# j-wilson/GPflowPILCO

Measured on AMD Instinct MI355X. Metric: moment_matched_rollout_step_elements_per_sec, higher is better.
Workload: dtype f32; 1 GPU; C3 (BASELINE configs[2]): N=2000 d=8 D=8 H=40 fp32 drift moment-match step / closed rollout; recipe=baseline: BASELINE.md recipe: lengthscales log-U[0.3,3], GP-prior targets, fresh mu~U[0,1]^d / Sigm~; N=2000, d=8, D=8, H=40, B_per_gpu=256, B_total=256, B_this_rank=256, parallelism=dp1 over B (weak), recipe=baseline, steps_requested=418, diag_pairs=f64, offdiag_pairs=f32

## Files before the change

gpflowpilco_amd/_lib.py:

```python
from __future__ import annotations

import ctypes as C
import os

_HERE = os.path.dirname(os.path.abspath(__file__))
LIB_PATH = os.environ.get("GPFLOWPILCO_MM_LIB") or os.path.join(_HERE, "libgpflowpilco_mm.so")

MM_F32, MM_F64 = 0, 1
MM_DMAX = 32
MM_M_ALIGN = 128
MM_FULL_OUTPUT_COV = 1
MM_MODEL_UNCERTAINTY = 2
MM_FORCE_GENERIC = 4
MM_STAGE_DIAG = 8
MM_STAGE_OFFDIAG = 16
MM_STAGE_FINALIZE = 32
MM_FORCE_WORST_TIER = 64
MM_WORKSPACE_CURRENT = 128
MM_FORCE_ROUTE = 256
MM_NO_ROUTE = 512
MM_SUMS_CURRENT = 1024
MM_ISTAGE_OLD_SKIP_BOUND = 1 << 26
MM_ISTAGE_NO_BOUND_SKIP = 1 << 27

ERRORS = {
    -1: "MM_E_ARG: NULL pointer or non-positive size",
    -2: "MM_E_DIM: input dimension d exceeds MM_DMAX=32 or unsupported shape",
    -3: "MM_E_DTYPE: dtype must be MM_F32 or MM_F64",
    -4: "MM_E_WORKSPACE: workspace/packed buffer too small",
    -5: "MM_E_NO_C: model_uncertainty requested but the model was packed without C",
    -6: "MM_E_STATE: Euler update / closed rollout needs d == L and a full output covariance",
}

SIGNATURES = {
    "mm_abi_version": (C.c_int, []),
    "mm_packed_model_bytes": (C.c_size_t, [C.c_int] * 5),
    "mm_pack_model": (C.c_int, [C.c_void_p, C.c_size_t, C.c_int, C.c_int, C.c_int, C.c_int]
                      + [C.c_void_p] * 6 + [C.c_void_p]),
    "mm_pack_perm": (C.c_int, [C.c_void_p, C.c_size_t, C.c_int, C.c_int, C.c_int, C.c_int, C.c_void_p, C.c_void_p]),
    "mm_workspace_bytes": (C.c_size_t, [C.c_int] * 6),
    "mm_moment_match": (C.c_int, [C.c_void_p, C.c_size_t, C.c_int, C.c_int, C.c_int, C.c_int, C.c_int,
                                  C.c_void_p, C.c_void_p, C.c_int, C.c_double,
                                  C.c_void_p, C.c_void_p, C.c_void_p,
                                  C.c_void_p, C.c_size_t, C.c_void_p, C.c_void_p]),
    "mm_q_forward": (C.c_int, [C.c_void_p, C.c_size_t, C.c_int, C.c_int, C.c_int, C.c_int, C.c_int,
                               C.c_void_p, C.c_void_p, C.c_int,
                               C.c_void_p, C.c_void_p, C.c_void_p,
                               C.c_void_p, C.c_size_t, C.c_void_p, C.c_void_p]),
    "mm_Q_reduce_forward": (C.c_int, [C.c_void_p, C.c_size_t, C.c_int, C.c_int, C.c_int, C.c_int, C.c_int,
                                      C.c_int, C.c_double, C.c_void_p,
                                      C.c_void_p, C.c_size_t, C.c_void_p]),
    "mm_euler_update": (C.c_int, [C.c_int, C.c_int, C.c_int, C.c_double] + [C.c_void_p] * 8),
    "mm_expected_cost": (C.c_int, [C.c_int, C.c_int, C.c_int] + [C.c_void_p] * 6),
    "mm_offdiag_stats": (C.c_int, [C.c_void_p, C.c_size_t, C.c_int, C.c_int, C.c_int, C.c_int, C.c_int, C.c_int,
                                   C.c_void_p, C.c_size_t, C.c_void_p, C.c_void_p]),
    "mm_offdiag_worklist_len": (C.c_int, [C.c_int] * 6 + [C.c_void_p, C.c_size_t, C.c_void_p, C.c_void_p]),
    "mm_offdiag_skip_bounds": (C.c_int, [C.c_void_p, C.c_size_t, C.c_int, C.c_int, C.c_int, C.c_int, C.c_int, C.c_int,
                                         C.c_void_p, C.c_size_t, C.c_void_p, C.c_void_p, C.c_void_p]),
    "mm_route_estimates": (C.c_int, [C.c_void_p, C.c_size_t, C.c_int, C.c_int, C.c_int, C.c_int, C.c_int, C.c_int,
                                     C.c_void_p, C.c_size_t, C.c_void_p, C.c_void_p]),
    "mm_compose_workspace_bytes": (C.c_size_t, [C.c_int] * 4),
    "mm_compose_nd_workspace_bytes": (C.c_size_t, [C.c_int] * 5),
    "mm_compose_tape_bytes": (C.c_size_t, [C.c_int] * 6),
    "mm_compose_backward_workspace_bytes": (C.c_size_t, [C.c_int] * 4),
    "mm_policy_grad_bytes": (C.c_size_t, [C.c_int] * 3),
    "mm_compose_tape_bytes_nd": (C.c_size_t, [C.c_int] * 7),
    "mm_compose_backward_workspace_bytes_nd": (C.c_size_t, [C.c_int] * 6),
    "mm_policy_grad_bytes_nd": (C.c_size_t, [C.c_int] * 4),
    "mm_compose_nd_mixed_workspace_bytes": (C.c_size_t, [C.c_int] * 6),
    "mm_compose_tape_bytes_nd_mixed": (C.c_size_t, [C.c_int] * 8),
    "mm_compose_backward_workspace_bytes_nd_mixed": (C.c_size_t, [C.c_int] * 7),
    "mm_bwd_f32_supported": (C.c_int, [C.c_int]),
    "mm_backward_pair_aggregates_bytes": (C.c_size_t, [C.c_int] * 5),
    "mm_backward_pair_aggregates": (C.c_int, [C.c_void_p, C.c_size_t, C.c_int, C.c_int, C.c_int, C.c_int, C.c_int,
                                              C.c_void_p, C.c_void_p, C.c_int, C.c_void_p, C.c_size_t, C.c_void_p, C.c_size_t,
                                              C.c_void_p, C.c_size_t, C.c_void_p, C.c_void_p]),
    "mm_moment_match_backward_bytes": (C.c_size_t, [C.c_int] * 5),
    "mm_moment_match_backward_bytes_dtype": (C.c_size_t, [C.c_int] * 6),
    "mm_moment_match_backward": (C.c_int, [C.c_void_p, C.c_size_t, C.c_int, C.c_int, C.c_int, C.c_int, C.c_int,
                                           C.c_void_p, C.c_void_p, C.c_int,
                                           C.c_void_p, C.c_void_p, C.c_void_p,
                                           C.c_void_p, C.c_void_p, C.c_int,
                                           C.c_void_p, C.c_size_t, C.c_void_p, C.c_size_t,
                                           C.c_void_p, C.c_void_p]),
    "mm_moment_match_with_sums": (C.c_int, [C.c_void_p, C.c_size_t, C.c_int, C.c_int, C.c_int, C.c_int, C.c_int,
                                            C.c_void_p, C.c_void_p, C.c_int, C.c_double,
                                            C.c_void_p, C.c_void_p, C.c_void_p,
                                            C.c_void_p, C.c_size_t, C.c_void_p, C.c_size_t,
                                            C.c_void_p, C.c_void_p]),
    "mm_backward_bytes": (C.c_size_t, [C.c_int] * 5),
    "mm_backward_sums": (C.c_int, [C.c_void_p, C.c_size_t, C.c_int, C.c_int, C.c_int, C.c_int, C.c_int,
                                   C.c_void_p, C.c_int, C.c_void_p, C.c_size_t, C.c_void_p, C.c_size_t, C.c_void_p]),
    "mm_pathwise_eval": (C.c_int, [C.c_int] * 6 + [C.c_void_p] * 12),
    "mm_pathwise_rollout": (C.c_int, [C.c_int] * 7 + [C.c_double] + [C.c_void_p] * 13),
    "mm_pathwise_eval_jac": (C.c_int, [C.c_int] * 6 + [C.c_void_p] * 13),
    "mm_pathwise_eval_bound": (C.c_int, [C.c_int] * 6 + [C.c_void_p] * 13),
    "mm_pathwise_tape_bytes": (C.c_size_t, [C.c_int] * 6),
    "mm_pathwise_policy_rollout": (C.c_int, [C.c_int] * 5 + [C.c_double, C.c_int, C.c_int] + [C.c_void_p] * 10
                                   + [C.c_void_p, C.c_size_t, C.c_int, C.c_double, C.c_double]
                                   + [C.c_void_p] * 4 + [C.c_void_p, C.c_size_t, C.c_int, C.c_void_p]),
    "mm_pathwise_backward_scratch_bytes": (C.c_size_t, [C.c_int] * 3),
    "mm_pathwise_policy_rollout_backward": (C.c_int, [C.c_int] * 3 + [C.c_double, C.c_int, C.c_int, C.c_void_p]
                                            + [C.c_void_p, C.c_size_t, C.c_int, C.c_double, C.c_double]
                                            + [C.c_void_p] * 2 + [C.c_void_p, C.c_size_t] + [C.c_void_p] * 3
                                            + [C.c_void_p, C.c_size_t, C.c_void_p]),
    "mm_pathwise_policy_rollout_backward_seeded": (C.c_int, [C.c_int] * 3 + [C.c_double, C.c_int, C.c_int, C.c_void_p]
                                                   + [C.c_void_p, C.c_size_t, C.c_int, C.c_double, C.c_double]
                                                   + [C.c_void_p] * 2 + [C.c_void_p, C.c_size_t] + [C.c_void_p] * 4
                                                   + [C.c_void_p, C.c_size_t, C.c_void_p]),
    "mm_pathwise_tape_bytes_nd": (C.c_size_t, [C.c_int] * 7),
    "mm_pathwise_policy_rollout_nd": (C.c_int, [C.c_int] * 5 + [C.c_double, C.c_int, C.c_int, C.c_void_p, C.c_int]
                                      + [C.c_void_p] * 9
                                      + [C.c_void_p, C.c_size_t, C.c_int, C.c_void_p, C.c_void_p]
                                      + [C.c_void_p] * 4 + [C.c_void_p, C.c_size_t, C.c_int, C.c_void_p]),
    "mm_pathwise_backward_scratch_bytes_nd": (C.c_size_t, [C.c_int] * 4),
    "mm_pathwise_policy_rollout_backward_nd": (C.c_int, [C.c_int] * 3 + [C.c_double, C.c_int, C.c_int, C.c_void_p, C.c_int]
                                               + [C.c_void_p, C.c_size_t, C.c_int, C.c_void_p, C.c_void_p]
                                               + [C.c_void_p] * 2 + [C.c_void_p, C.c_size_t] + [C.c_void_p] * 3
                                               + [C.c_void_p, C.c_size_t, C.c_void_p]),
    "mm_pathwise_policy_rollout_backward_nd_seeded": (C.c_int, [C.c_int] * 3 + [C.c_double, C.c_int, C.c_int, C.c_void_p, C.c_int]
                                                      + [C.c_void_p, C.c_size_t, C.c_int, C.c_void_p, C.c_void_p]
                                                      + [C.c_void_p] * 2 + [C.c_void_p, C.c_size_t] + [C.c_void_p] * 4
                                                      + [C.c_void_p, C.c_size_t, C.c_void_p]),
    "mm_pathwise_policy_rollout_wide": (C.c_int, [C.c_int] * 5 + [C.c_double, C.c_int, C.c_int, C.c_void_p, C.c_int]
                                        + [C.c_void_p] * 9
                                        + [C.c_void_p, C.c_size_t, C.c_int, C.c_void_p, C.c_void_p]
                                        + [C.c_void_p] * 4 + [C.c_void_p, C.c_size_t, C.c_int, C.c_void_p]),
    "mm_pathwise_backward_scratch_bytes_wide": (C.c_size_t, [C.c_int] * 4),
    "mm_pathwise_policy_rollout_backward_wide": (C.c_int, [C.c_int] * 3 + [C.c_double, C.c_int, C.c_int, C.c_void_p, C.c_int]
                                                 + [C.c_void_p, C.c_size_t, C.c_int, C.c_void_p, C.c_void_p]
                                                 + [C.c_void_p] * 2 + [C.c_void_p, C.c_size_t] + [C.c_void_p] * 3
                                                 + [C.c_void_p, C.c_size_t, C.c_void_p]),
    "mm_pathwise_policy_rollout_backward_wide_seeded": (C.c_int, [C.c_int] * 3 + [C.c_double, C.c_int, C.c_int, C.c_void_p, C.c_int]
                                                        + [C.c_void_p, C.c_size_t, C.c_int, C.c_void_p, C.c_void_p]
                                                        + [C.c_void_p] * 2 + [C.c_void_p, C.c_size_t] + [C.c_void_p] * 4
                                                        + [C.c_void_p, C.c_size_t, C.c_void_p]),
    "mm_pathwise_tape_bytes_mixed": (C.c_size_t, [C.c_int] * 8),
    "mm_pathwise_policy_rollout_mixed": (C.c_int, [C.c_int] * 5 + [C.c_double, C.c_int, C.c_int, C.c_void_p, C.c_int]
                                         + [C.c_void_p] * 9
                                         + [C.c_void_p, C.c_size_t, C.c_int, C.c_void_p, C.c_void_p]
                                         + [C.c_void_p] * 4 + [C.c_void_p, C.c_size_t, C.c_int, C.c_void_p]
                                         + [C.c_int, C.c_void_p, C.c_void_p]),
    "mm_pathwise_policy_rollout_backward_mixed": (C.c_int, [C.c_int] * 3 + [C.c_double, C.c_int, C.c_int, C.c_void_p, C.c_int]
                                                  + [C.c_void_p, C.c_size_t, C.c_int, C.c_void_p, C.c_void_p]
                                                  + [C.c_void_p] * 2 + [C.c_void_p, C.c_size_t] + [C.c_void_p] * 4
                                                  + [C.c_void_p, C.c_size_t, C.c_void_p] + [C.c_int, C.c_void_p]),
    "mm_pathwise_eval_kern": (C.c_int, [C.c_int] * 6 + [C.c_void_p] * 12 + [C.c_int]),
    "mm_pathwise_rollout_kern": (C.c_int, [C.c_int] * 7 + [C.c_double] + [C.c_void_p] * 13 + [C.c_int]),
    "mm_pathwise_eval_jac_kern": (C.c_int, [C.c_int] * 6 + [C.c_void_p] * 13 + [C.c_int]),
    "mm_pathwise_eval_bound_kern": (C.c_int, [C.c_int] * 6 + [C.c_void_p] * 13 + [C.c_int]),
    "mm_pathwise_policy_rollout_kern": (C.c_int, [C.c_int] * 5 + [C.c_double, C.c_int, C.c_int, C.c_void_p, C.c_int]
                                        + [C.c_void_p] * 9
                                        + [C.c_void_p, C.c_size_t, C.c_int, C.c_void_p, C.c_void_p]
                                        + [C.c_void_p] * 4 + [C.c_void_p, C.c_size_t, C.c_int, C.c_void_p]
                                        + [C.c_int, C.c_void_p, C.c_void_p, C.c_int]),
    "mm_pathwise_mean_eval": (C.c_int, [C.c_int] * 5 + [C.c_void_p] * 10 + [C.c_int]),
    "mm_pathwise_policy_rollout_mean": (C.c_int, [C.c_int] * 4 + [C.c_double, C.c_int, C.c_int, C.c_void_p, C.c_int]
                                        + [C.c_void_p] * 6
                                        + [C.c_void_p, C.c_size_t, C.c_int, C.c_void_p, C.c_void_p]
                                        + [C.c_void_p] * 4 + [C.c_void_p, C.c_size_t, C.c_int, C.c_void_p]
                                        + [C.c_int, C.c_void_p, C.c_void_p, C.c_int]),
    "mm_pathwise_basis": (C.c_int, [C.c_int] * 5 + [C.c_void_p] * 9),
    "mm_pathwise_pack_stream": (C.c_int, [C.c_int] * 5 + [C.c_void_p] * 4),
    "mm_gram_workspace_bytes": (C.c_size_t, [C.c_int] * 4),
    "mm_gram_se": (C.c_int, [C.c_int] * 4 + [C.c_void_p] * 6),
    "mm_gram_se_backward": (C.c_int, [C.c_int] * 4 + [C.c_void_p] * 9 + [C.c_size_t, C.c_void_p]),
    "mm_predict_workspace_bytes": (C.c_size_t, [C.c_int] * 4),
    "mm_predict_se": (C.c_int, [C.c_int] * 4 + [C.c_void_p] * 10 + [C.c_size_t, C.c_void_p]),
    "mm_rollout_closed": (C.c_int, [C.c_void_p, C.c_size_t, C.c_int, C.c_int, C.c_int, C.c_int, C.c_int, C.c_int,
                                    C.c_double, C.c_int, C.c_double,
                                    C.c_void_p, C.c_void_p, C.c_void_p, C.c_void_p,
                                    C.c_void_p, C.c_size_t, C.c_void_p, C.c_void_p]),
}


def _composed_rollout_signatures():
# ... 65 lines not shown
```

gpflowpilco_amd/csrc/mm_common.h:

```cpp
#pragma once
#include <stddef.h>
#include <stdint.h>
#include "../../include/gpflowpilco_mm.h"

static inline size_t mm_align_up(size_t x, size_t a) { return (x + a - 1) / a * a; }
static inline int mm_round_up_int(int x, int a) { return (x + a - 1) / a * a; }
static inline size_t mm_elem_size(int dtype) { return dtype == MM_F64 ? 8 : 4; }

#define MM_ISTAGE_NO_ROUTE (1 << 20)
#define MM_ISTAGE_ROUTE (1 << 21)
#define MM_ISTAGE_NO_M56 (1 << 22)
#define MM_ISTAGE_OLD_OFFDIAG (1 << 23)
#define MM_ISTAGE_OLD_SPOLY56 (1 << 24)
#define MM_ISTAGE_OLD_DIAG_MAP (1 << 25)
#define MM_ISTAGE_OLD_SKIP_BOUND (1 << 26)
#define MM_ISTAGE_NO_BOUND_SKIP (1 << 27)

#define MM_PW_KERNELS 3

static inline int mm_num_pairs(int L, int flags) {
  return (flags & MM_FULL_OUTPUT_COV) ? L * (L + 1) / 2 : L;
}

static inline int mm_moment_deg(int d) { return d <= 8 ? 4 : 2; }
static inline long long mm_binom(int n, int k) {
  if (k < 0 || k > n) return 0;
  long long r = 1;
  for (int i = 1; i <= k; ++i) r = r * (n - k + i) / i;
  return r;
}
static inline int mm_mono_count(int n, int d) { return (int)mm_binom(d + n - 1, n); }
static inline int mm_mono_offset(int n, int d) { int o = 0; for (int m = 0; m < n; ++m) o += mm_mono_count(m, d); return o; }
static inline size_t mm_rank_table_entries(int d) {
  const int dk = d <= 8 ? 8 : 32, deg = mm_moment_deg(d);
  size_t n = 0, p = 1;
  for (int k = 1; k <= deg; ++k) { p *= dk; n += p; }
  return n;
}
static inline int mm_moment_cols(int d) { return mm_round_up_int(mm_mono_offset(mm_moment_deg(d) + 1, d), 16); }
static inline int mm_moment56_off5(int d) { return d <= 8 ? mm_round_up_int(mm_mono_count(4, d), 128) : 0; }
static inline int mm_moment56_off6(int d) { return d <= 8 ? mm_moment56_off5(d) + mm_round_up_int(mm_mono_count(5, d), 128) : 0; }
static inline int mm_moment56_cols(int d) { return d <= 8 ? mm_moment56_off6(d) + mm_round_up_int(mm_mono_count(6, d), 128) : 0; }
struct MMTab56 { int ins[6], last[6], n_i16, mult2, mult3, n_f32; size_t bytes; };
static inline MMTab56 mm_tab56(int d) {
  MMTab56 t;
  int o = 0;
  for (int m = 0; m < 6; ++m) { t.ins[m] = o; o += mm_mono_count(m, d) * 8; }
  for (int k = 0; k < 6; ++k) { t.last[k] = o; o += mm_mono_count(k, d); }
  t.n_i16 = mm_round_up_int(o, 8);
  t.mult2 = 0; t.mult3 = mm_mono_count(2, d); t.n_f32 = mm_mono_count(2, d) + mm_mono_count(3, d);
  t.bytes = (size_t)t.n_i16 * 2 + (size_t)t.n_f32 * 4;
  return t;
}

struct MMModelLayout {
  int Mp, Kz, nd8, KMp;
  size_t Z64;
  size_t Zt64;
  size_t zbar;
  size_t ls2;
  size_t var;
  size_t meanc;
  size_t beta64;
  size_t Zc64;
  size_t Zc;
  size_t Zs3;
  size_t Zm;
  size_t zmax2;
  size_t rtab;
  size_t Zq2;
  size_t Zm56;
  size_t tab56;
  size_t perm;
  size_t skey;
  size_t zt2;
  size_t zt2s;
  size_t Cm;
  size_t total;
};
#define MM_SORT_MIN_M 256

static inline MMModelLayout mm_model_layout(int L, int M, int d, int dtype, int with_C) {
  MMModelLayout o;
  const size_t es = mm_elem_size(dtype), A = 256;
  o.Mp = mm_round_up_int(M, MM_M_ALIGN);
  o.Kz = mm_round_up_int(d, 2);
  o.nd8 = (d + 7) / 8;
  o.KMp = mm_moment_cols(d);
  size_t off = 0;
  o.Z64 = off;    off = mm_align_up(off + (size_t)L * M * d * 8, A);
  o.Zt64 = off;   off = mm_align_up(off + (size_t)L * d * o.Mp * 8, A);
  o.zbar = off;   off = mm_align_up(off + (size_t)L * d * 8, A);
  o.ls2 = off;    off = mm_align_up(off + (size_t)L * d * 8, A);
  o.var = off;    off = mm_align_up(off + (size_t)L * 8, A);
  o.meanc = off;  off = mm_align_up(off + (size_t)L * 8, A);
  o.beta64 = off; off = mm_align_up(off + (size_t)L * M * 8, A);
  o.Zc64 = off;   off = mm_align_up(off + (size_t)L * o.Mp * o.Kz * 8, A);
  o.Zc = o.Zc64;
  if (dtype != MM_F64) { o.Zc = off; off = mm_align_up(off + (size_t)L * o.Mp * o.Kz * es, A); }
  o.Zs3 = off;
  if (dtype != MM_F64) off = mm_align_up(off + (size_t)L * o.Mp * 24 * o.nd8 * 2, A);
  o.Zm = off;
  if (dtype != MM_F64) off = mm_align_up(off + (size_t)L * o.Mp * o.KMp * 8, A);
  o.zmax2 = off;  off = mm_align_up(off + (size_t)L * 8, A);
  o.rtab = off;   off = mm_align_up(off + mm_rank_table_entries(d) * 2, A);
  o.Zq2 = off;
  if (dtype != MM_F64 && d <= 8) off = mm_align_up(off + (size_t)L * (o.Mp / 32) * 8192, A);
  o.Zm56 = off;
  if (dtype != MM_F64 && d <= 8) off = mm_align_up(off + (size_t)L * 2 * mm_moment56_cols(d) * o.Mp * 2, A);
  o.tab56 = off;
  if (dtype != MM_F64 && d <= 8) off = mm_align_up(off + mm_tab56(d).bytes, A);
  o.perm = off;   off = mm_align_up(off + (size_t)L * o.Mp * 4, A);
  o.skey = off;   off = mm_align_up(off + (size_t)L * o.Mp * 8, A);
  o.zt2 = off;    off = mm_align_up(off + (size_t)L * (o.Mp / 32) * 4, A);
  o.zt2s = off;   off = mm_align_up(off + (size_t)L * (o.Mp / 32) * 4, A);
  o.Cm = off;
  if (with_C) off = mm_align_up(off + (size_t)L * o.Mp * o.Mp * 8, A);
  o.total = off;
  return o;
}

#define MM_MOM_SPLIT 2
#ifndef MM_COLLAPSE_BOUND2
#define MM_COLLAPSE_BOUND2 0.25f
#endif
#define MM_C6_X5_2 (1.0f / 256.0f)
#define MM_C6_X4_2 (1.0f / 1600.0f)
#define MM_C6_MAX 0.25f
#define MM_C6_C0 1.666663289e-01f
#define MM_C6_C1 4.166659713e-02f
#define MM_C6_C2 8.350561373e-03f
#define MM_C6_C3 1.391559141e-03f
#define MM_C6_SYS2 6.33e-6f
#define MM_C6_POLY_F64(x_) (((x_) * (x_)) * (x_) * fma(fma(fma((double)MM_C6_C3, (x_), (double)MM_C6_C2), (x_), (double)MM_C6_C1), (x_), (double)MM_C6_C0))
#ifndef MM_TIER1_DIV
#define MM_TIER1_DIV 20
#endif
#if MM_TIER1_DIV == 16
#define MM_TIER1_MAX 0.0625f
#define MM_REM1_C0 1.666936278e-01f
#define MM_REM1_C1 4.167173430e-02f
#elif MM_TIER1_DIV == 20
#define MM_TIER1_MAX 0.05f
#define MM_REM1_C0 1.666839272e-01f
#define MM_REM1_C1 4.166988656e-02f
#elif MM_TIER1_DIV == 24
#define MM_TIER1_MAX 0.041666668f
#define MM_REM1_C0 1.666786522e-01f
#define MM_REM1_C1 4.166889191e-02f
#elif MM_TIER1_DIV == 32
#define MM_TIER1_MAX 0.03125f
#define MM_REM1_C0 1.666734070e-01f
#define MM_REM1_C1 4.166791216e-02f
#else
#error "MM_TIER1_DIV must be 16, 20, 24 or 32"
#endif
#define MM_INSIDE_BOUND2 (0.998f * MM_C6_MAX * MM_C6_MAX)
#ifndef MM_ROUTE_TOL
#define MM_ROUTE_TOL 3.0e-4
#endif
#define MM_ROUTE_CSPLIT 8
static inline int mm_route_ncc(int NS, int npanel) { int n = NS / npanel; return n < 1 ? 1 : (n > MM_ROUTE_CSPLIT ? MM_ROUTE_CSPLIT : n); }
#define MM_EXP_CAP_F64 700.0
#define MM_EXP_CAP_F32 80.0f
#define MM_GEN_ROWS 64
#define MM_GEN_COLS 256
#define MM_PANEL_ROWS 256
__host__ __device__ inline int mm_mfma_groups(int Mp) { return (Mp + MM_PANEL_ROWS - 1) / MM_PANEL_ROWS * (MM_PANEL_ROWS / 64); }
__host__ __device__ inline int mm_f32p_list_off(int L) { return 4 + 2 * L; }
// ... 109 lines not shown
```

gpflowpilco_amd/csrc/mm_moments.hip:

```cpp
#include <hip/hip_runtime.h>
#include <math.h>
#include "mm_common.h"
#include "mm_mono.h"

typedef double f64x4m __attribute__((ext_vector_type(4)));

#define MM_GEMM_RB 64
#define MM_GEMM_NB 128
#define MM_GEMM_KB 32
#define MM_GEMM_AS 34
#define MM_GEMM_BS 144

__device__ __forceinline__ void mm_decode_pair_m(int p, int L, int& a, int& a2) {
  int r = p - L, i = 0;
  while (r >= L - 1 - i) { r -= L - 1 - i; ++i; }
  a = i; a2 = i + 1 + r;
}

__global__ __launch_bounds__(256) __attribute__((amdgpu_waves_per_eu(2, 2))) void k_wmom_gemm(const double* __restrict__ whR, const double* __restrict__ whC,
                                                      const double* __restrict__ Zm, int KMp, int L, int Mp, int B, int Po,
                                                      int nrb, int ncb, int nwork, int col_deg3,
                                                      const unsigned int* __restrict__ amaxc, const double* __restrict__ zmax2,
                                                      const int* __restrict__ gperm, double* __restrict__ mom) {
  const int orig = blockIdx.x;
  const int xcd = orig & 7, slot = orig >> 3;
  const int qn = nwork >> 3, rn = nwork & 7;
  int wi = (xcd < rn ? xcd * (qn + 1) : rn * (qn + 1) + (xcd - rn) * qn) + slot;
  const int rb = wi % nrb; wi /= nrb;
  const int ks = wi % MM_MOM_SPLIT; wi /= MM_MOM_SPLIT;
  const int cb = wi % ncb; wi /= ncb;
  const int a = wi;
  const int R = (L - 1) * B;
  auto row_item = [&](int r, int& b, int& po, int& side, int& acol) {
    const int which = r / B;
    b = r - which * B;
    const int ap = which < a ? which : which + 1;
    const int lo = ap < a ? ap : a, hi = ap < a ? a : ap;
    po = lo * (L - 1) - lo * (lo - 1) / 2 + (hi - lo - 1);
    side = ap < a ? 1 : 0;
    acol = hi;
  };
  const double* tab = Zm + (size_t)a * Mp * KMp;
  const int tid = threadIdx.x, wv = tid >> 6, lane = tid & 63, l15 = lane & 15, kq = lane >> 4;
  const int* perm = nullptr;
  if (cb * MM_GEMM_NB >= col_deg3) {
    if (gperm != nullptr) {
      if (rb * MM_GEMM_RB >= gperm[(size_t)L * R + a]) return;
      perm = gperm + (size_t)a * R;
    } else {
      const int r = rb * MM_GEMM_RB + lane;
      bool c = false;
      if (amaxc != nullptr && r < R) {
        int b, po, side, acol;
        row_item(r, b, po, side, acol);
        c = mm_item_collapsed(amaxc[(size_t)b * Po + po]);
      }
      if (!__any(c)) return;
    }
  }
  const int kslice = Mp / MM_MOM_SPLIT;
  const int k_begin = ks * kslice, nkb = kslice / MM_GEMM_KB;

  __shared__ double As[MM_GEMM_RB * MM_GEMM_AS];
  __shared__ double Bs[MM_GEMM_KB * MM_GEMM_BS];

  const int ar = tid >> 2, ak = (tid & 3) * 8;
  int arow = rb * MM_GEMM_RB + ar;
  arow = arow < R ? arow : R - 1;
  int ab, apo, aside, aacol;
  row_item(perm ? perm[arow] : arow, ab, apo, aside, aacol);
  const double* aptr = (aside ? whC : whR) + ((size_t)ab * Po + apo) * Mp + k_begin + ak;

  const int bk = tid >> 3, bc = (tid & 7) * 16;
  const int col0 = cb * MM_GEMM_NB + bc;
  const bool bvalid = col0 < KMp;
  const double* bptr = tab + (size_t)(k_begin + bk) * KMp + (bvalid ? col0 : 0);
  double2 ra[4], rbv[8];
  auto load_regs = [&](int kb) {
    const double* ap = aptr + kb * MM_GEMM_KB;
#pragma unroll
    for (int i = 0; i < 4; ++i) ra[i] = *reinterpret_cast<const double2*>(ap + 2 * i);
    const double* bp = bptr + (size_t)kb * MM_GEMM_KB * KMp;
#pragma unroll
    for (int i = 0; i < 8; ++i) rbv[i] = *reinterpret_cast<const double2*>(bp + 2 * i);
  };
  f64x4m acc[4][2];
#pragma unroll
  for (int rt = 0; rt < 4; ++rt)
#pragma unroll
    for (int ct = 0; ct < 2; ++ct) acc[rt][ct] = (f64x4m){0.0, 0.0, 0.0, 0.0};

  load_regs(0);
  for (int kb = 0; kb < nkb; ++kb) {
    __syncthreads();
#pragma unroll
    for (int i = 0; i < 4; ++i) *reinterpret_cast<double2*>(&As[ar * MM_GEMM_AS + ak + 2 * i]) = ra[i];
#pragma unroll
    for (int i = 0; i < 8; ++i)
      *reinterpret_cast<double2*>(&Bs[bk * MM_GEMM_BS + bc + 2 * ((i + (tid & 7)) & 7)]) = bvalid ? rbv[i] : make_double2(0.0, 0.0);
    __syncthreads();
    load_regs(kb + 1 < nkb ? kb + 1 : kb);
#pragma unroll
    for (int s = 0; s < MM_GEMM_KB / 4; ++s) {
      double av[4], bv[2];
#pragma unroll
      for (int rt = 0; rt < 4; ++rt) av[rt] = As[(rt * 16 + l15) * MM_GEMM_AS + 4 * s + kq];
#pragma unroll
      for (int ct = 0; ct < 2; ++ct)
        bv[ct] = Bs[(4 * s + kq) * MM_GEMM_BS + wv * 32 + ct * 16 + 2 * (((l15 >> 1) + 2 * wv + ct) & 7) + (l15 & 1)];
#pragma unroll
      for (int rt = 0; rt < 4; ++rt)
#pragma unroll
        for (int ct = 0; ct < 2; ++ct)
          acc[rt][ct] = __builtin_amdgcn_mfma_f64_16x16x4f64(av[rt], bv[ct], acc[rt][ct], 0, 0, 0);
    }
  }
#pragma unroll
  for (int rt = 0; rt < 4; ++rt)
#pragma unroll
    for (int r = 0; r < 4; ++r) {
      const int row = rb * MM_GEMM_RB + rt * 16 + kq + 4 * r;
      if (row >= R) continue;
      int b, po, side, acol;
      row_item(perm ? perm[row] : row, b, po, side, acol);
      double* o = mom + ((((size_t)b * Po + po) * 2 + side) * MM_MOM_SPLIT + ks) * KMp;
#pragma unroll
      for (int ct = 0; ct < 2; ++ct) {
        const int col = cb * MM_GEMM_NB + wv * 32 + ct * 16 + l15;
        if (col < KMp) o[col] = acc[rt][ct][r];
      }
    }
}

__global__ __launch_bounds__(1024) void k_wmom_perm(const unsigned int* __restrict__ amaxc, const double* __restrict__ zmax2, int L, int B,
                                                    int Po, int* __restrict__ gperm) {
  const int a = blockIdx.x, tid = threadIdx.x, wv = tid >> 6, lane = tid & 63;
  const int R = (L - 1) * B;
  __shared__ int wsum[3][16];
  __shared__ int tot[3];
  int* out = gperm + (size_t)a * R;
  int cnt[3] = {0, 0, 0};
  auto cls_of = [&](int r) {
    const int which = r / B, b = r - which * B;
    const int ap = which < a ? which : which + 1;
    const int lo = ap < a ? ap : a, hi = ap < a ? a : ap;
    const int po = lo * (L - 1) - lo * (lo - 1) / 2 + (hi - lo - 1);
    const unsigned int ac = amaxc[(size_t)b * Po + po];
    const float x2 = mm_collapse_bound2(ac, zmax2[hi]);
    return !mm_item_collapsed(ac) ? 3 : (x2 > MM_C6_X5_2 ? 0 : (x2 > MM_C6_X4_2 ? 1 : 2));
  };
  for (int r = tid; r < R; r += 1024) { const int c = cls_of(r); if (c < 3) ++cnt[c]; }
#pragma unroll
  for (int c = 0; c < 3; ++c) {
#pragma unroll
    for (int off = 32; off > 0; off >>= 1) cnt[c] += __shfl_down(cnt[c], off, 64);
    if (lane == 0) wsum[c][wv] = cnt[c];
  }
  __syncthreads();
  if (tid < 3) { int t = 0; for (int w = 0; w < 16; ++w) t += wsum[tid][w]; tot[tid] = t; }
  __syncthreads();
  int ofs[3] = {0, tot[0], tot[0] + tot[1]};
  int ofs_n = 0;
  for (int r0 = 0; r0 < R; r0 += 1024) {
    const int r = r0 + tid;
    const bool in = r < R;
    const int c = in ? cls_of(r) : 4;
    int before[3], ctot[3];
    __syncthreads();
#pragma unroll
    for (int k = 0; k < 3; ++k) {
      const unsigned long long bal = __ballot(c == k);
      before[k] = __popcll(bal & ((1ull << lane) - 1ull));
      if (lane == 0) wsum[k][wv] = __popcll(bal);
    }
    __syncthreads();
    int nfront_before = 0, nfront_tot = 0;
#pragma unroll
    for (int k = 0; k < 3; ++k) {
      int wb = 0, ct = 0;
#pragma unroll
      for (int w = 0; w < 16; ++w) { if (w < wv) wb += wsum[k][w]; ct += wsum[k][w]; }
      before[k] += wb; ctot[k] = ct;
      nfront_before += before[k]; nfront_tot += ct;
    }
    if (in) {
      if (c < 3) out[ofs[c] + before[c]] = r;
      else out[R - 1 - (ofs_n + (tid - nfront_before))] = r;
    }
    const int nin = R - r0 < 1024 ? R - r0 : 1024;
#pragma unroll
    for (int k = 0; k < 3; ++k) ofs[k] += ctot[k];
    ofs_n += nin - nfront_tot;
  }
  if (tid == 0) {
    gperm[(size_t)L * R + a] = tot[0] + tot[1] + tot[2];
    gperm[(size_t)L * R + L + a] = tot[0] + tot[1];
    gperm[(size_t)L * R + 2 * L + a] = tot[0];
  }
}

__device__ __forceinline__ double mm_block_sum256m(double v, double* red) {
#pragma unroll
  for (int off = 32; off > 0; off >>= 1) v += __shfl_down(v, off, 64);
  __syncthreads();
  if ((threadIdx.x & 63) == 0) red[threadIdx.x >> 6] = v;
  __syncthreads();
  return red[0] + red[1] + red[2] + red[3];
}

template <int DK, int LB>
__global__ __launch_bounds__(256) void k_spoly(const double* __restrict__ mom, int KMp, const double* __restrict__ pairmat,
                                               const double* __restrict__ zbar, const double* __restrict__ zmax2,
                                               const unsigned int* __restrict__ amax, const unsigned int* __restrict__ amaxc,
                                               const float* __restrict__ mu,
                                               int L, int d, int P, int deg, int allow_collapse,
                                               int off1, int off2, int off3, int off4, const short* __restrict__ rtab,
                                               double c0, double c1, double* __restrict__ s12) {
  extern __shared__ double sm[];
  const int po = blockIdx.x, b = blockIdx.y, tid = threadIdx.x;
  const int Po = P - L, p = L + po;
  int a, a2;
  mm_decode_pair_m(p, L, a, a2);
  const int dn = 1 << (LB * deg);
#define MM_PADI(i_) ((i_) + ((i_) >> 5))
  double* T = sm;
  double* U = T + MM_PADI(dn);
  double* nh = U + MM_PADI(dn >> LB);
  double* qh = nh + KMp;
  double* Gs = qh + KMp;
  double* dmu = Gs + DK * DK;
  __shared__ double red[4];
  {
    const double* nm = mom + (((size_t)b * Po + po) * 2 + 0) * MM_MOM_SPLIT * KMp;
    const double* qm = mom + (((size_t)b * Po + po) * 2 + 1) * MM_MOM_SPLIT * KMp;
    for (int k = tid; k < KMp; k += 256) {
      double sn = 0.0, sq = 0.0;
#pragma unroll
      for (int t = 0; t < MM_MOM_SPLIT; ++t) { sn += nm[t * KMp + k]; sq += qm[t * KMp + k]; }
      nh[k] = sn; qh[k] = sq;
    }
    const double* pm = pairmat + ((size_t)b * P + p) * (d * d + 1);
    for (int idx = tid; idx < DK * DK; idx += 256) {
      const int i = idx >> LB, j = idx & (DK - 1);
      Gs[idx] = (i < d && j < d) ? pm[i * d + j] : 0.0;
    }
    const bool rcen = mm_rows_recentred(amax[(size_t)b * Po + po]);
    if (tid < DK) dmu[tid] = (tid < d && !rcen) ? (double)mu[(size_t)b * d + tid] - zbar[a * d + tid] : 0.0;
  }
  __syncthreads();
  const bool coll = allow_collapse && deg >= 3 && mm_item_collapsed(amaxc[(size_t)b * Po + po]);
  const int nmax = coll ? deg : 2;
  double Gr[DK == 8 ? 64 : 1];
  if constexpr (DK == 8) {
#pragma unroll
    for (int i = 0; i < 64; ++i) Gr[i] = Gs[i];
  }
  double total = 0.0;
  for (int n = nmax; n >= 1; --n) {
    const double an = n == 1 ? 1.0 : n == 2 ? 0.5 : n == 3 ? c0 : c1;
    const int dsz = 1 << (LB * n);
    const int offn = n == 1 ? off1 : n == 2 ? off2 : n == 3 ? off3 : off4;
    const short* rtn = rtab + (((1 << (LB * n)) - DK) / (DK - 1));
    for (int idx = tid; idx < dsz; idx += 256) {
      const int r = rtn[idx];
      T[MM_PADI(idx)] = r >= 0 ? qh[offn + r] : 0.0;
    }
    __syncthreads();
    for (int t = 0; t < n; ++t) {
      const int sh = LB * t, nfib = dsz >> LB;
      for (int f = tid; f < nfib; f += 256) {
        const int lo = f & ((1 << sh) - 1), hi = f >> sh;
        const int base = (hi << (sh + LB)) + lo;
        double v[DK];
#pragma unroll
        for (int l = 0; l < DK; ++l) v[l] = T[MM_PADI(base + (l << sh))];
        if constexpr (DK == 8) {
#pragma unroll
          for (int k = 0; k < 8; ++k) {
            double s = 0.0;
#pragma unroll
            for (int l = 0; l < 8; ++l) s = fma(Gr[k * 8 + l], v[l], s);
            T[MM_PADI(base + (k << sh))] = s;
          }
        } else {
#pragma unroll 2
          for (int k = 0; k < DK; ++k) {
            double s = 0.0;
#pragma unroll
            for (int l = 0; l < DK; ++l) s = fma(Gs[k * DK + l], v[l], s);
            T[MM_PADI(base + (k << sh))] = s;
          }
        }
      }
      __syncthreads();
    }
    double* cur = T;
    double* oth = U;
    int ksz = dsz;
    double sign_binom = 1.0;
    for (int k = n; k >= 0; --k) {
      const int offk = k == 0 ? 0 : k == 1 ? off1 : k == 2 ? off2 : k == 3 ? off3 : off4;
      double part = 0.0;
      const short* rtk = rtab + (k ? (((1 << (LB * k)) - DK) / (DK - 1)) : 0);
      for (int idx = tid; idx < ksz; idx += 256) {
        const int r = k ? rtk[idx] : 0;
        if (r >= 0) part = fma(cur[MM_PADI(idx)], nh[offk + r], part);
      }
      total = fma(an * sign_binom, part, total);
      if (k == 0) break;
      const int nsz = ksz >> LB;
      for (int idx = tid; idx < nsz; idx += 256) {
        double s = 0.0;
#pragma unroll
        for (int l = 0; l < DK; ++l) s = fma(cur[MM_PADI(l * nsz + idx)], dmu[l], s);
        oth[MM_PADI(idx)] = s;
      }
      __syncthreads();
      double* tsw = cur; cur = oth; oth = tsw;
      ksz = nsz;
      sign_binom = -sign_binom * (double)k / (double)(n - k + 1);
    }
    __syncthreads();
  }
  const double tot = mm_block_sum256m(total, red);
  if (tid == 0) s12[(size_t)b * Po + po] = tot + nh[0] * qh[0];
#undef MM_PADI
}

int mm_launch_wmom_full(const char* packed, const MMModelLayout& ml, char* ws, const MMWorkspaceLayout& wl,
                        int B, int L, int d, hipStream_t stream) {
  const int nrb = ((L - 1) * B + MM_GEMM_RB - 1) / MM_GEMM_RB, ncb = (ml.KMp + MM_GEMM_NB - 1) / MM_GEMM_NB;
  const long long nwork_ll = (long long)L * ncb * MM_MOM_SPLIT * nrb;
  if (nwork_ll <= 0 || nwork_ll > 0x7fffffffLL) return MM_E_DIM;
  hipLaunchKernelGGL(k_wmom_gemm, dim3((int)nwork_ll), dim3(256), 0, stream, (const double*)(ws + wl.whR),
                     (const double*)(ws + wl.whC), (const double*)(packed + ml.Zm), ml.KMp, L, wl.Mp, B, wl.Po, nrb, ncb,
                     (int)nwork_ll, 0x7fffffff , (const unsigned int*)nullptr, (const double*)(packed + ml.zmax2),
                     (const int*)nullptr, (double*)(ws + wl.mom));
  hipError_t e = hipGetLastError();
  return e == hipSuccess ? 0 : (int)e;
}

int mm_launch_moments56(const char* packed, const MMModelLayout& ml, char* ws, const MMWorkspaceLayout& wl,
                        int B, int L, int d, int allow, int old_spoly56, hipStream_t stream);

int mm_launch_moments(const char* packed, const MMModelLayout& ml, char* ws, const MMWorkspaceLayout& wl,
                      int B, int L, int d, const void* mu_f32, int flags, hipStream_t stream) {
  const double* Zm = (const double*)(packed + ml.Zm);
  double* mom = (double*)(ws + wl.mom);
  const int deg = mm_moment_deg(d) >= 4 ? 3 : mm_moment_deg(d);
  const int ncol_fwd = mm_mono_offset(deg + 1, d);
  const int nrb = ((L - 1) * B + MM_GEMM_RB - 1) / MM_GEMM_RB, ncb = (ncol_fwd + MM_GEMM_NB - 1) / MM_GEMM_NB;
  const long long nwork_ll = (long long)L * ncb * MM_MOM_SPLIT * nrb;
  if (nwork_ll <= 0 || nwork_ll > 0x7fffffffLL) return MM_E_DIM;
  const int nwork = (int)nwork_ll;
  const int allow = (flags & (MM_FORCE_WORST_TIER | MM_ISTAGE_NO_M56)) ? 0 : 1;
  const int col_deg3 = mm_mono_offset(3, d);
  const bool some = allow && mm_moment_deg(d) >= 4;
  if (some) {
    hipLaunchKernelGGL(k_wmom_perm, dim3(L), dim3(1024), 0, stream, (const unsigned int*)(ws + wl.amaxc),
                       (const double*)(packed + ml.zmax2), L, B, wl.Po, (int*)(ws + wl.gperm));
    hipError_t ep = hipGetLastError();
    if (ep != hipSuccess) return (int)ep;
  }
  hipLaunchKernelGGL(k_wmom_gemm, dim3(nwork), dim3(256), 0, stream, (const double*)(ws + wl.whR),
                     (const double*)(ws + wl.whC), Zm, ml.KMp, L, wl.Mp, B, wl.Po, nrb, ncb, nwork, col_deg3,
                     some ? (const unsigned int*)(ws + wl.amaxc) : (const unsigned int*)nullptr,
                     (const double*)(packed + ml.zmax2), some ? (const int*)(ws + wl.gperm) : (const int*)nullptr, mom);
  hipError_t e = hipGetLastError();
  if (e != hipSuccess) return (int)e;
  const int off1 = mm_mono_offset(1, d), off2 = mm_mono_offset(2, d), off3 = mm_mono_offset(3, d), off4 = mm_mono_offset(4, d);
#define MM_SPOLY(DK_, LB_)                                                                                                       \
  do {                                                                                                                          \
    const int dn_ = 1 << (LB_ * deg);                                                                                           \
    const int up_ = dn_ >> LB_;                                                                                                 \
    const size_t shm_ = (size_t)(dn_ + (dn_ >> 5) + up_ + (up_ >> 5) + 2 * ml.KMp + DK_ * DK_ + DK_ + 8) * sizeof(double);      \
    hipLaunchKernelGGL((k_spoly<DK_, LB_>), dim3(wl.Po, B), dim3(256), shm_, stream, (const double*)mom, ml.KMp,                \
                       (const double*)(ws + wl.pairmat), (const double*)(packed + ml.zbar), (const double*)(packed + ml.zmax2), \
                       (const unsigned int*)(ws + wl.amax), (const unsigned int*)(ws + wl.amaxc), (const float*)mu_f32, L, d, wl.P, deg, allow, off1, off2, off3, off4, \
                       (const short*)(packed + ml.rtab),                                                                        \
                       (double)MM_C6_C0, (double)MM_C6_C1, (double*)(ws + wl.s12));                                             \
  } while (0)
  if (d <= 8) MM_SPOLY(8, 3); else MM_SPOLY(32, 5);
#undef MM_SPOLY
  e = hipGetLastError();
  if (e != hipSuccess) return (int)e;
  if (flags & MM_ISTAGE_NO_M56) {
    if (mm_moment56_cols(d) <= 0 || wl.Po <= 0) return 0;
    const hipError_t em = hipMemsetAsync(ws + wl.s56, 0xFF, (size_t)B * wl.Po * sizeof(double), stream);
    if (em != hipSuccess) return (int)em;
    const hipError_t es = hipMemsetAsync(ws + wl.estS, 0, (size_t)B * wl.Po * sizeof(float), stream);
    return es == hipSuccess ? 0 : (int)es;
  }
  return mm_launch_moments56(packed, ml, ws, wl, B, L, d, some ? 1 : 0, (flags & MM_ISTAGE_OLD_SPOLY56) ? 1 : 0, stream);
}

__global__ void k_offdiag_stats(const unsigned int* __restrict__ amax, const double* __restrict__ zmax2,
                                const unsigned char* __restrict__ gflag, int ng, int L, int Po, int n,
                                int32_t* __restrict__ out) {
  const int idx = blockIdx.x * blockDim.x + threadIdx.x;
  bool c = false, in = false, part = false;
  int groups = 0;
  if (idx < n) {
    int a, a2;
    mm_decode_pair_m(L + idx % Po, L, a, a2);
    const float b2 = mm_collapse_bound2(amax[idx], zmax2[a2]);
    c = b2 <= MM_COLLAPSE_BOUND2;
    in = b2 <= MM_INSIDE_BOUND2;
    part = !c && mm_item_collapsed(amax[n + idx]);
    for (int g = 0; g < ng; ++g) groups += gflag[(size_t)idx * ng + g] ? 1 : 0;
  }
  const unsigned long long m = __ballot(c), mi = __ballot(in), mp = __ballot(part);
  if ((threadIdx.x & 63) == 0 && m) atomicAdd(out, (int)__popcll(m));
  if ((threadIdx.x & 63) == 0 && mi) atomicAdd(out + 2, (int)__popcll(mi));
  if ((threadIdx.x & 63) == 0 && mp) atomicAdd(out + 4, (int)__popcll(mp));
#pragma unroll
  for (int off = 32; off > 0; off >>= 1) groups += __shfl_down(groups, off, 64);
  if ((threadIdx.x & 63) == 0 && groups) atomicAdd(out + 5, groups);
  if (idx == 0) out[1] = n;
}

extern "C" int mm_offdiag_stats(const void* packed, size_t packed_bytes, int L, int M, int d, int dtype, int B, int flags,
                                const void* workspace, size_t workspace_bytes, int32_t* out, void* stream) {
  if (!packed || !workspace || !out || L <= 0 || M <= 0 || d <= 0 || d > MM_DMAX || B <= 0) return MM_E_ARG;
  const MMModelLayout ml = mm_model_layout(L, M, d, dtype, 1);
  const MMWorkspaceLayout wl = mm_workspace_layout(B, L, M, d, dtype, flags);
  if (packed_bytes < ml.Cm || workspace_bytes < wl.total) return MM_E_WORKSPACE;
  hipStream_t s = (hipStream_t)stream;
  hipError_t e = hipMemsetAsync(out, 0, 6 * sizeof(int32_t), s);
  if (e != hipSuccess) return (int)e;
  if (dtype == MM_F32 && wl.Po > 0) {
    e = hipMemcpyAsync(out + 3, (const char*)workspace + wl.rcount + 4, sizeof(int32_t), hipMemcpyDeviceToDevice, s);
    if (e != hipSuccess) return (int)e;
  }
  if (dtype != MM_F32 || wl.Po == 0 || mm_moment_deg(d) < 4 || (flags & MM_FORCE_WORST_TIER)) return 0;
  const int n = B * wl.Po;
  hipLaunchKernelGGL(k_offdiag_stats, dim3((n + 255) / 256), dim3(256), 0, s, (const unsigned int*)((const char*)workspace + wl.amax),
                     (const double*)((const char*)packed + ml.zmax2), (const unsigned char*)((const char*)workspace + wl.gflag),
                     wl.Mp / MM_GROUP_ROWS, L, wl.Po, n, out);
  e = hipGetLastError();
  return e == hipSuccess ? 0 : (int)e;
}
```

Measured before the change: 45530 rollout step-elements/s (B*H per rollout second).

## Add one-pass wide-column moment GEMM and wave-per-item spoly kernel

Replaces the column-blocked f64 MFMA moment GEMM with a templated variant in which each workgroup covers all needed column tiles (up to 11×16) in one pass. Each A row tile is then loaded once instead of once per column block. A per-permutation split lets collapsed rows use fewer tiles. It also replaces the block-per-item k_spoly for d<=8 with a kernel that gives each item one wavefront, holds G in registers and syncs with wave-level barriers instead of block-level ones. The cost is more register and LDS pressure and many template instantiations. The old path stays reachable through a new flag.

Result: faster. 46630 rollout step-elements/s (B*H per rollout second) (median of 6 runs) (+2.4%).

```diff
diff --git a/gpflowpilco_amd/_lib.py b/gpflowpilco_amd/_lib.py
--- a/gpflowpilco_amd/_lib.py
+++ b/gpflowpilco_amd/_lib.py
@@ -22,6 +22,7 @@
 MM_SUMS_CURRENT = 1024
 MM_ISTAGE_OLD_SKIP_BOUND = 1 << 26
 MM_ISTAGE_NO_BOUND_SKIP = 1 << 27
+MM_ISTAGE_OLD_WMOM = 1 << 28
 
 ERRORS = {
     -1: "MM_E_ARG: NULL pointer or non-positive size",
diff --git a/gpflowpilco_amd/csrc/mm_common.h b/gpflowpilco_amd/csrc/mm_common.h
--- a/gpflowpilco_amd/csrc/mm_common.h
+++ b/gpflowpilco_amd/csrc/mm_common.h
@@ -15,6 +15,7 @@
 #define MM_ISTAGE_OLD_DIAG_MAP (1 << 25)
 #define MM_ISTAGE_OLD_SKIP_BOUND (1 << 26)
 #define MM_ISTAGE_NO_BOUND_SKIP (1 << 27)
+#define MM_ISTAGE_OLD_WMOM (1 << 28)
 
 #define MM_PW_KERNELS 3
 
diff --git a/gpflowpilco_amd/csrc/mm_moments.hip b/gpflowpilco_amd/csrc/mm_moments.hip
--- a/gpflowpilco_amd/csrc/mm_moments.hip
+++ b/gpflowpilco_amd/csrc/mm_moments.hip
@@ -4,6 +4,7 @@
 #include "mm_mono.h"
 
 typedef double f64x4m __attribute__((ext_vector_type(4)));
+typedef double f64x2m __attribute__((ext_vector_type(2)));
 
 #define MM_GEMM_RB 64
 #define MM_GEMM_NB 128
@@ -132,6 +133,112 @@
     }
 }
 
+#define MM_GEMM1_MAXT 11
+#define MM_GEMM1_BS(NT_) ((NT_) * 16 + (((NT_) & 1) ? 0 : 16))
+#define MM_GEMM1_LDS(NT_) ((size_t)(MM_GEMM_RB * MM_GEMM_AS + MM_GEMM_KB * MM_GEMM1_BS(NT_)) * sizeof(double))
+
+template <int NT, class OutRow>
+__device__ __forceinline__ void mm_wmom_rows(const double* __restrict__ aptr, const double* __restrict__ bptr, int KMp, int nkb,
+                                             double* __restrict__ As, double* __restrict__ Bs, int tid, OutRow&& out_row) {
+  constexpr int BS = MM_GEMM1_BS(NT), W2 = NT * 8;
+  const int wv = tid >> 6, lane = tid & 63, l15 = lane & 15, kq = lane >> 4;
+  const int ar = tid >> 2, ak = (tid & 3) * 8;
+  int bsrc[NT], bdst[NT];
+#pragma unroll
+  for (int i = 0; i < NT; ++i) {
+    const int c = tid + 256 * i, row = c / W2, cp = c - row * W2;
+    bsrc[i] = row * KMp + 2 * cp;
+    bdst[i] = row * BS + 2 * cp;
+  }
+  f64x2m ra[4], rbv[NT];
+  f64x4m acc[NT];
+#define MM_G1_LOAD(kb_)                                                                                             \
+  do {                                                                                                              \
+    const double* ap_ = aptr + (kb_) * MM_GEMM_KB;                                                                  \
+    _Pragma("unroll") for (int i = 0; i < 4; ++i) ra[i] = *reinterpret_cast<const f64x2m*>(ap_ + 2 * i);           \
+    const double* bp_ = bptr + (size_t)(kb_) * MM_GEMM_KB * KMp;                                                    \
+    _Pragma("unroll") for (int i = 0; i < NT; ++i) rbv[i] = *reinterpret_cast<const f64x2m*>(bp_ + bsrc[i]);       \
+  } while (0)
+#pragma unroll
+  for (int ct = 0; ct < NT; ++ct) acc[ct] = (f64x4m){0.0, 0.0, 0.0, 0.0};
+  MM_G1_LOAD(0);
+  for (int kb = 0; kb < nkb; ++kb) {
+    __syncthreads();
+#pragma unroll
+    for (int i = 0; i < 4; ++i) *reinterpret_cast<f64x2m*>(&As[ar * MM_GEMM_AS + ak + 2 * i]) = ra[i];
+#pragma unroll
+    for (int i = 0; i < NT; ++i) *reinterpret_cast<f64x2m*>(&Bs[bdst[i]]) = rbv[i];
+    __syncthreads();
+    MM_G1_LOAD(kb + 1 < nkb ? kb + 1 : kb);
+#pragma unroll
+    for (int s = 0; s < MM_GEMM_KB / 4; ++s) {
+      const double av = As[(wv * 16 + l15) * MM_GEMM_AS + 4 * s + kq];
+      double bv[NT];
+#pragma unroll
+      for (int ct = 0; ct < NT; ++ct) bv[ct] = Bs[(4 * s + kq) * BS + ct * 16 + l15];
+#pragma unroll
+      for (int ct = 0; ct < NT; ++ct) acc[ct] = __builtin_amdgcn_mfma_f64_16x16x4f64(av, bv[ct], acc[ct], 0, 0, 0);
+    }
+  }
+#pragma unroll
+  for (int r = 0; r < 4; ++r) {
+    double* o = out_row(r);
+    if (o == nullptr) continue;
+#pragma unroll
+    for (int ct = 0; ct < NT; ++ct) o[ct * 16] = acc[ct][r];
+  }
+#undef MM_G1_LOAD
+}
+
+template <int NT_HI, int NT_LO>
+__global__ __launch_bounds__(256) __attribute__((amdgpu_waves_per_eu(2, 2))) void k_wmom_gemm1(
+    const double* __restrict__ whR, const double* __restrict__ whC, const double* __restrict__ Zm, int KMp, int L, int Mp, int B,
+    int Po, int nrb, int nwork, int col0, const int* __restrict__ gperm, double* __restrict__ mom) {
+  static_assert(NT_LO <= NT_HI && NT_HI <= MM_GEMM1_MAXT, "column tiles per workgroup");
+  const int orig = blockIdx.x;
+  const int xcd = orig & 7, slot = orig >> 3;
+  const int qn = nwork >> 3, rn = nwork & 7;
+  int wi = (xcd < rn ? xcd * (qn + 1) : rn * (qn + 1) + (xcd - rn) * qn) + slot;
+  const int ks = wi % MM_MOM_SPLIT; wi /= MM_MOM_SPLIT;
+  const int rb = wi % nrb; wi /= nrb;
+  const int a = wi;
+  const int R = (L - 1) * B;
+  auto row_item = [&](int r, int& b, int& po, int& side) {
+    const int which = r / B;
+    b = r - which * B;
+    const int ap = which < a ? which : which + 1;
+    const int lo = ap < a ? ap : a, hi = ap < a ? a : ap;
+    po = lo * (L - 1) - lo * (lo - 1) / 2 + (hi - lo - 1);
+    side = ap < a ? 1 : 0;
+  };
+  const int* perm = gperm != nullptr ? gperm + (size_t)a * R : nullptr;
+  const bool all_tiles = NT_LO == NT_HI || rb * MM_GEMM_RB < gperm[(size_t)L * R + a];
+  const int tid = threadIdx.x, wv = tid >> 6, lane = tid & 63, l15 = lane & 15, kq = lane >> 4;
+  const int kslice = Mp / MM_MOM_SPLIT;
+  const int k_begin = ks * kslice, nkb = kslice / MM_GEMM_KB;
+
+  extern __shared__ double sm_g1[];
+  double* As = sm_g1;
+  double* Bs = sm_g1 + MM_GEMM_RB * MM_GEMM_AS;
+
+  int arow = rb * MM_GEMM_RB + (tid >> 2);
+  arow = arow < R ? arow : R - 1;
+  int ab, apo, aside;
+  row_item(perm ? perm[arow] : arow, ab, apo, aside);
+  const double* aptr = (aside ? whC : whR) + ((size_t)ab * Po + apo) * Mp + k_begin + (tid & 3) * 8;
+  const double* bptr = Zm + ((size_t)a * Mp + k_begin) * KMp + col0;
+
+  auto out_row = [&](int r) -> double* {
+    const int row = rb * MM_GEMM_RB + wv * 16 + kq + 4 * r;
+    if (row >= R) return nullptr;
+    int b, po, side;
+    row_item(perm ? perm[row] : row, b, po, side);
+    return mom + ((((size_t)b * Po + po) * 2 + side) * MM_MOM_SPLIT + ks) * KMp + col0 + l15;
+  };
+  if (all_tiles) mm_wmom_rows<NT_HI>(aptr, bptr, KMp, nkb, As, Bs, tid, out_row);
+  else mm_wmom_rows<NT_LO>(aptr, bptr, KMp, nkb, As, Bs, tid, out_row);
+}
+
 __global__ __launch_bounds__(1024) void k_wmom_perm(const unsigned int* __restrict__ amaxc, const double* __restrict__ zmax2, int L, int B,
                                                     int Po, int* __restrict__ gperm) {
   const int a = blockIdx.x, tid = threadIdx.x, wv = tid >> 6, lane = tid & 63;
@@ -327,6 +434,134 @@
 #undef MM_PADI
 }
 
+#define MM_SPW_WAVES 4
+__device__ __forceinline__ void mm_wave_sync_m() {
+  __builtin_amdgcn_fence(__ATOMIC_RELEASE, "wavefront");
+  __builtin_amdgcn_wave_barrier();
+  __builtin_amdgcn_fence(__ATOMIC_ACQUIRE, "wavefront");
+}
+static inline int mm_spw_slice(int ncs) { return 512 + 16 + 64 + 2 + 2 * ncs + 64 + 8; }
+
+__global__ __launch_bounds__(64 * MM_SPW_WAVES) void k_spoly_wave8(const double* __restrict__ mom, int KMp, const double* __restrict__ pairmat,
+                                                                   const double* __restrict__ zbar, const unsigned int* __restrict__ amax,
+                                                                   const unsigned int* __restrict__ amaxc, const float* __restrict__ mu,
+                                                                   int L, int d, int P, int B, int allow_collapse,
+                                                                   int off1, int off2, int off3, int off4, int ncs, int slice,
+                                                                   const short* __restrict__ rtab, double c0,
+                                                                   double* __restrict__ s12) {
+  constexpr int DK = 8, LB = 3, DEG = 3;
+  extern __shared__ double sm[];
+  const int lane = threadIdx.x & 63, wv = threadIdx.x >> 6;
+  const int Po = P - L;
+  const int item = blockIdx.x * MM_SPW_WAVES + wv;
+  if (item >= B * Po) return;
+  const int b = item / Po, po = item - b * Po, p = L + po;
+  int a, a2;
+  mm_decode_pair_m(p, L, a, a2);
+  constexpr int dn = 1 << (LB * DEG);
+#define MM_PADI(i_) ((i_) + ((i_) >> 5))
+  double* T = sm + (size_t)wv * slice;
+  double* U = T + MM_PADI(dn);
+  double* nh = U + MM_PADI(dn >> LB);
+  double* qh = nh + ncs;
+  double* Gs = qh + ncs;
+  double* dmu = Gs + DK * DK;
+  const bool coll = allow_collapse && mm_item_collapsed(amaxc[(size_t)b * Po + po]);
+  const int nmax = coll ? DEG : 2;
+  {
+    const int ncol = coll ? off4 : off3;
+    const double* nm = mom + (((size_t)b * Po + po) * 2 + 0) * MM_MOM_SPLIT * KMp;
+    const double* qm = mom + (((size_t)b * Po + po) * 2 + 1) * MM_MOM_SPLIT * KMp;
+    for (int k = lane; k < ncol; k += 64) {
+      double sn = 0.0, sq = 0.0;
+#pragma unroll
+      for (int t = 0; t < MM_MOM_SPLIT; ++t) { sn += nm[t * KMp + k]; sq += qm[t * KMp + k]; }
+      nh[k] = sn; qh[k] = sq;
+    }
+    const double* pm = pairmat + ((size_t)b * P + p) * (d * d + 1);
+    {
+      const int i = lane >> LB, j = lane & (DK - 1);
+      Gs[lane] = (i < d && j < d) ? pm[i * d + j] : 0.0;
+    }
+    const bool rcen = mm_rows_recentred(amax[(size_t)b * Po + po]);
+    if (lane < DK) dmu[lane] = (lane < d && !rcen) ? (double)mu[(size_t)b * d + lane] - zbar[a * d + lane] : 0.0;
+  }
+  mm_wave_sync_m();
+  double Gr[64];
+#pragma unroll
+  for (int i = 0; i < 64; ++i) Gr[i] = Gs[i];
+  double total[4] = {0.0, 0.0, 0.0, 0.0};
+  for (int n = nmax; n >= 1; --n) {
+    const double an = n == 1 ? 1.0 : n == 2 ? 0.5 : c0;
+    const int dsz = 1 << (LB * n);
+    const int offn = n == 1 ? off1 : n == 2 ? off2 : off3;
+    const short* rtn = rtab + (((1 << (LB * n)) - DK) / (DK - 1));
+    for (int idx = lane; idx < dsz; idx += 64) {
+      const int r = rtn[idx];
+      T[MM_PADI(idx)] = r >= 0 ? qh[offn + r] : 0.0;
+    }
+    mm_wave_sync_m();
+    for (int t = 0; t < n; ++t) {
+      const int sh = LB * t, nfib = dsz >> LB;
+      for (int f = lane; f < nfib; f += 64) {
+        const int lo = f & ((1 << sh) - 1), hi = f >> sh;
+        const int base = (hi << (sh + LB)) + lo;
+        double v[DK];
+#pragma unroll
+        for (int l = 0; l < DK; ++l) v[l] = T[MM_PADI(base + (l << sh))];
+#pragma unroll
+        for (int k = 0; k < 8; ++k) {
+          double s = 0.0;
+#pragma unroll
+          for (int l = 0; l < 8; ++l) s = fma(Gr[k * 8 + l], v[l], s);
+          T[MM_PADI(base + (k << sh))] = s;
+        }
+      }
+      mm_wave_sync_m();
+    }
+    double* cur = T;
+    double* oth = U;
+    int ksz = dsz;
+    double sign_binom = 1.0;
+    for (int k = n; k >= 0; --k) {
+      const int offk = k == 0 ? 0 : k == 1 ? off1 : k == 2 ? off2 : off3;
+      const short* rtk = rtab + (k ? (((1 << (LB * k)) - DK) / (DK - 1)) : 0);
+#pragma unroll
+      for (int v = 0; v < 4; ++v) {
+        double part = 0.0;
+        for (int idx = lane + 64 * v; idx < ksz; idx += 256) {
+          const int r = k ? rtk[idx] : 0;
+          if (r >= 0) part = fma(cur[MM_PADI(idx)], nh[offk + r], part);
+        }
+        total[v] = fma(an * sign_binom, part, total[v]);
+      }
+      if (k == 0) break;
+      const int nsz = ksz >> LB;
+      for (int idx = lane; idx < nsz; idx += 64) {
+        double s = 0.0;
+#pragma unroll
+        for (int l = 0; l < DK; ++l) s = fma(cur[MM_PADI(l * nsz + idx)], dmu[l], s);
+        oth[MM_PADI(idx)] = s;
+      }
+      mm_wave_sync_m();
+      double* tsw = cur; cur = oth; oth = tsw;
+      ksz = nsz;
+      sign_binom = -sign_binom * (double)k / (double)(n - k + 1);
+    }
+    mm_wave_sync_m();
+  }
+#pragma unroll
+  for (int v = 0; v < 4; ++v) {
+#pragma unroll
+    for (int off = 32; off > 0; off >>= 1) total[v] += __shfl_down(total[v], off, 64);
+  }
+  if (lane == 0) {
+    const double tot = total[0] + total[1] + total[2] + total[3];
+    s12[(size_t)b * Po + po] = tot + nh[0] * qh[0];
+  }
+#undef MM_PADI
+}
+
 int mm_launch_wmom_full(const char* packed, const MMModelLayout& ml, char* ws, const MMWorkspaceLayout& wl,
                         int B, int L, int d, hipStream_t stream) {
   const int nrb = ((L - 1) * B + MM_GEMM_RB - 1) / MM_GEMM_RB, ncb = (ml.KMp + MM_GEMM_NB - 1) / MM_GEMM_NB;
@@ -338,6 +573,38 @@
                      (const int*)nullptr, (double*)(ws + wl.mom));
   hipError_t e = hipGetLastError();
   return e == hipSuccess ? 0 : (int)e;
+}
+
+typedef void (*mm_gemm1_fn)(const double*, const double*, const double*, int, int, int, int, int, int, int, int, const int*, double*);
+static mm_gemm1_fn mm_gemm1_kernel(int hi, int lo) {
+#define MM_G1(HI_, LO_) if (hi == HI_ && lo == LO_) return k_wmom_gemm1<HI_, LO_>
+  MM_G1(1, 1); MM_G1(2, 2); MM_G1(3, 3); MM_G1(4, 4); MM_G1(5, 5); MM_G1(6, 6); MM_G1(7, 7); MM_G1(8, 8); MM_G1(9, 9);
+  MM_G1(10, 10); MM_G1(11, 11);
+  MM_G1(2, 1); MM_G1(3, 1); MM_G1(4, 2); MM_G1(6, 2); MM_G1(8, 3); MM_G1(11, 3);
+#undef MM_G1
+  return nullptr;
+}
+
+static int mm_launch_wmom_onepass(const char* packed, const MMModelLayout& ml, char* ws, const MMWorkspaceLayout& wl, int B, int L,
+                                  int ncol, int col_deg3, const int* gperm, hipStream_t stream) {
+  const int nrb = ((L - 1) * B + MM_GEMM_RB - 1) / MM_GEMM_RB;
+  const long long nwork_ll = (long long)L * MM_MOM_SPLIT * nrb;
+  if (nwork_ll <= 0 || nwork_ll > 0x7fffffffLL) return MM_E_DIM;
+  const int nt = (ncol + 15) / 16;
+  const int npass = gperm != nullptr ? 1 : (nt + MM_GEMM1_MAXT - 1) / MM_GEMM1_MAXT;
+  const int per = (nt + npass - 1) / npass;
+  for (int p = 0; p < npass; ++p) {
+    const int hi = nt - p * per < per ? nt - p * per : per;
+    const int lo = gperm != nullptr ? (col_deg3 + 15) / 16 : hi;
+    const mm_gemm1_fn fn = mm_gemm1_kernel(hi, lo < hi ? lo : hi);
+    if (fn == nullptr || 16 * (p * per + hi) > ml.KMp) return MM_E_DIM;
+    hipLaunchKernelGGL(fn, dim3((int)nwork_ll), dim3(256), MM_GEMM1_LDS(hi), stream, (const double*)(ws + wl.whR), (const double*)(ws + wl.whC),
+                       (const double*)(packed + ml.Zm), ml.KMp, L, wl.Mp, B, wl.Po, nrb, (int)nwork_ll, 16 * p * per, gperm,
+                       (double*)(ws + wl.mom));
+    const hipError_t e = hipGetLastError();
+    if (e != hipSuccess) return (int)e;
+  }
+  return 0;
 }
 
 int mm_launch_moments56(const char* packed, const MMModelLayout& ml, char* ws, const MMWorkspaceLayout& wl,
@@ -362,12 +629,21 @@
     hipError_t ep = hipGetLastError();
     if (ep != hipSuccess) return (int)ep;
   }
-  hipLaunchKernelGGL(k_wmom_gemm, dim3(nwork), dim3(256), 0, stream, (const double*)(ws + wl.whR),
-                     (const double*)(ws + wl.whC), Zm, ml.KMp, L, wl.Mp, B, wl.Po, nrb, ncb, nwork, col_deg3,
-                     some ? (const unsigned int*)(ws + wl.amaxc) : (const unsigned int*)nullptr,
-                     (const double*)(packed + ml.zmax2), some ? (const int*)(ws + wl.gperm) : (const int*)nullptr, mom);
-  hipError_t e = hipGetLastError();
-  if (e != hipSuccess) return (int)e;
+  const bool old_wmom = (flags & MM_ISTAGE_OLD_WMOM) != 0;
+  hipError_t e = hipSuccess;
+  if (old_wmom) {
+    hipLaunchKernelGGL(k_wmom_gemm, dim3(nwork), dim3(256), 0, stream, (const double*)(ws + wl.whR),
+                       (const double*)(ws + wl.whC), Zm, ml.KMp, L, wl.Mp, B, wl.Po, nrb, ncb, nwork, col_deg3,
+                       some ? (const unsigned int*)(ws + wl.amaxc) : (const unsigned int*)nullptr,
+                       (const double*)(packed + ml.zmax2), some ? (const int*)(ws + wl.gperm) : (const int*)nullptr, mom);
+    e = hipGetLastError();
+    if (e != hipSuccess) return (int)e;
+  } else {
+    const int ncol = (mm_moment_deg(d) >= 4 && !some) ? col_deg3 : ncol_fwd;
+    const int rc = mm_launch_wmom_onepass(packed, ml, ws, wl, B, L, ncol, col_deg3, some ? (const int*)(ws + wl.gperm) : (const int*)nullptr,
+                                          stream);
+    if (rc != 0) return rc;
+  }
   const int off1 = mm_mono_offset(1, d), off2 = mm_mono_offset(2, d), off3 = mm_mono_offset(3, d), off4 = mm_mono_offset(4, d);
 #define MM_SPOLY(DK_, LB_)                                                                                                       \
   do {                                                                                                                          \
@@ -380,7 +656,16 @@
                        (const short*)(packed + ml.rtab),                                                                        \
                        (double)MM_C6_C0, (double)MM_C6_C1, (double*)(ws + wl.s12));                                             \
   } while (0)
-  if (d <= 8) MM_SPOLY(8, 3); else MM_SPOLY(32, 5);
+  if (d <= 8 && !old_wmom) {
+    const int ncs = (off4 + 7) & ~7;
+    const int slice = mm_spw_slice(ncs);
+    const int nitem = B * wl.Po;
+    hipLaunchKernelGGL(k_spoly_wave8, dim3((nitem + MM_SPW_WAVES - 1) / MM_SPW_WAVES), dim3(64 * MM_SPW_WAVES),
+                       (size_t)MM_SPW_WAVES * slice * sizeof(double), stream, (const double*)mom, ml.KMp,
+                       (const double*)(ws + wl.pairmat), (const double*)(packed + ml.zbar), (const unsigned int*)(ws + wl.amax),
+                       (const unsigned int*)(ws + wl.amaxc), (const float*)mu_f32, L, d, wl.P, B, allow, off1, off2, off3, off4,
+                       ncs, slice, (const short*)(packed + ml.rtab), (double)MM_C6_C0, (double*)(ws + wl.s12));
+  } else if (d <= 8) MM_SPOLY(8, 3); else MM_SPOLY(32, 5);
 #undef MM_SPOLY
   e = hipGetLastError();
   if (e != hipSuccess) return (int)e;
```
